# manospits/parallel_heat

Hardware: AMD Instinct MI355X
Metric: Mcells/sec (whole node) + sec/1000 iters, 8192^2 grid at 1/2/4/8 MI355X (higher is better)
Workload: dtype fp32; 1 GPU; model=heat2d 5-point Jacobi (fixed boundary), grid=8192x8192, global_batch=1, seq_len=67108864, parallelism=domain-decomp 1x1 (local), tb_depth 12, halo 12, schedule sync, converge_check=False

## Files before the change

csrc/kernels/stencil.hip:

```cpp
#include <hip/hip_runtime.h>

#include <cmath>
#include <cstdlib>
#include <cstdio>
#include <cstring>
#include <iterator>
#include <map>
#include <mutex>
#include <string>
#include <tuple>
#include <vector>

#include "heat/common.hpp"
#include "heat/init_fn.hpp"
#include "heat/kernels.hpp"
#include "tb_common.hpp"
#include "tb_exp.hpp"
#include "tb_tile.hpp"

namespace heat::gpu {
namespace {

using tbdetail::in_interior;
using tbdetail::TbArgs;
using tbdetail::TbBox;
using tbdetail::wave_max_atomic;

__global__ void init_kernel(float* base, int64_t pitch, int64_t rows, int64_t hx, int64_t hy,
                            int64_t gx0, int64_t gy0, int64_t nx, int64_t ny, int mode,
                            uint64_t seed) {
  const int64_t c = int64_t(blockIdx.x) * blockDim.x + threadIdx.x;
  if (c >= pitch) return;
  for (int64_t r = blockIdx.y; r < rows; r += gridDim.y) {
    const int64_t gx = gx0 + r - hx, gy = gy0 + c - hy;
    base[r * pitch + c] = init_value(mode, gx, gy, nx, ny, seed);
  }
}

__global__ __launch_bounds__(256) void naive_kernel(const float* __restrict__ src,
                                                    float* __restrict__ dst, StencilGeom g,
                                                    Box box, unsigned* resid) {
  const int64_t c = box.c0 + int64_t(blockIdx.x) * 64 + threadIdx.x;
  const int64_t r = box.r0 + int64_t(blockIdx.y) * 4 + threadIdx.y;
  if (tbdetail::gated(g.gate)) return;
  unsigned m = 0;
  if (r < box.r1 && c < box.c1) {
    const int64_t i = r * g.pitch + c;
    const float v = src[i];
    float out = v;
    if (in_interior(g.gx0 + r, g.nx) && in_interior(g.gy0 + c, g.ny))
      out = g.numerics == 1
                ? stencil_mpi(v, src[i - g.pitch], src[i + g.pitch], src[i - 1], src[i + 1], g.cx, g.cy)
                : stencil(v, src[i - g.pitch], src[i + g.pitch], src[i - 1], src[i + 1], g.cx, g.cy);
    dst[i] = out;
    m = __float_as_uint(fabsf(out - v));
  }
  if (resid) wave_max_atomic(m, resid);
}

__global__ void pack_kernel(const float* __restrict__ origin, int64_t pitch, Box box,
                            float* __restrict__ buf) {
  const int64_t cols = box.c1 - box.c0, n = (box.r1 - box.r0) * cols;
  for (int64_t k = int64_t(blockIdx.x) * blockDim.x + threadIdx.x; k < n;
       k += int64_t(gridDim.x) * blockDim.x) {
    const int64_t r = k / cols, c = k % cols;
    buf[k] = origin[(box.r0 + r) * pitch + box.c0 + c];
  }
}

struct BoxCopies {
  BoxCopy c[kMaxBoxCopies];
};

__global__ __launch_bounds__(128) void box_copy_kernel(float* __restrict__ origin, int64_t pitch,
                                                       BoxCopies a, int to_buf) {
  const BoxCopy& c = a.c[blockIdx.y];
  const int64_t rows = c.box.r1 - c.box.r0, cols = c.box.c1 - c.box.c0;
  for (int64_t r = blockIdx.x; r < rows; r += gridDim.x) {
    float* f = origin + (c.box.r0 + r) * pitch + c.box.c0;
    float* b = c.buf + r * cols;
    for (int64_t j = threadIdx.x; j < cols; j += blockDim.x) {
      if (to_buf) b[j] = f[j];
      else f[j] = b[j];
    }
  }
}

__global__ void unpack_kernel(const float* __restrict__ buf, float* __restrict__ origin,
                              int64_t pitch, Box box) {
  const int64_t cols = box.c1 - box.c0, n = (box.r1 - box.r0) * cols;
  for (int64_t k = int64_t(blockIdx.x) * blockDim.x + threadIdx.x; k < n;
       k += int64_t(gridDim.x) * blockDim.x) {
    const int64_t r = k / cols, c = k % cols;
    origin[(box.r0 + r) * pitch + box.c0 + c] = buf[k];
  }
}

__global__ __launch_bounds__(256) void residual_kernel(const float* __restrict__ a,
                                                       const float* __restrict__ b,
                                                       int64_t pitch, Box box, unsigned* resid) {
  const int64_t c = box.c0 + int64_t(blockIdx.x) * 64 + threadIdx.x;
  unsigned m = 0;
  if (c < box.c1)
    for (int64_t r = box.r0 + blockIdx.y * 4 + threadIdx.y; r < box.r1; r += gridDim.y * 4)
      m = max(m, __float_as_uint(fabsf(a[r * pitch + c] - b[r * pitch + c])));
  wave_max_atomic(m, resid);
}

__global__ void judge_kernel(unsigned* resids, int n, int slots, int stride, DeviceGate* gate,
                             double eps, int mpi_compat) {
  constexpr int kMax = 32;
  const int lane = threadIdx.x;
  for (int i0 = 0; i0 < n; i0 += kMax) {
    const int m = min(n - i0, kMax);
    unsigned v[kMax];
#pragma unroll
    for (int j = 0; j < kMax; ++j) v[j] = (j < m && lane < slots) ? resids[lane * stride + i0 + j] : 0u;
#pragma unroll
    for (int j = 0; j < kMax; ++j)
      if (j < m && lane < slots) resids[lane * stride + i0 + j] = 0u;
    DeviceGate gl{};
    if (lane == 0) gl = *gate;
    for (int j = 0; j < m; ++j) {
      unsigned bits = v[j];
#pragma unroll
      for (int off = 32; off >= 1; off >>= 1) bits = max(bits, unsigned(__shfl_xor(int(bits), off)));
      if (lane == 0 && gl.stop == 0u) {
        float r;
        __builtin_memcpy(&r, &bits, 4);
        const unsigned ordinal = gl.checks;
        gl.checks = ordinal + 1u;
        gl.last_bits = bits;
        unsigned why = 0u;
        if ((bits & 0x7F800000u) == 0x7F800000u) why = 2u;
        else if (mpi_compat ? double(r) <= eps : r < float(eps)) why = 1u;
        if (why) {
          gl.reason = why;
          gl.stop_check = ordinal;
          gl.stop = 1u;
        }
      }
    }
    if (lane == 0) *gate = gl;
  }
}

__device__ __forceinline__ int float_key(float f) {
  const int i = __float_as_int(f);
  return i >= 0 ? i : (i ^ 0x7FFFFFFF);
}

__global__ __launch_bounds__(256) void checksum_kernel(const float* __restrict__ origin,
                                                       int64_t pitch, int64_t lx, int64_t ly,
                                                       int64_t ox, int64_t oy, int64_t ny,
                                                       DeviceChecksum* out) {
  unsigned long long h = 0, cnt = 0;
  double sum = 0.0;
  int mn = 0x7FFFFFFF, mx = int(0x80000000);
  for (int64_t r = blockIdx.y; r < lx; r += gridDim.y) {
    const float* row = origin + r * pitch;
    const uint64_t gbase = uint64_t(ox + r) * uint64_t(ny) + uint64_t(oy);
    for (int64_t c = int64_t(blockIdx.x) * blockDim.x + threadIdx.x; c < ly;
         c += int64_t(gridDim.x) * blockDim.x) {
      const float v = row[c];
      const uint32_t bits = __float_as_uint(v);
      h += mix64((gbase + uint64_t(c)) * 0x100000001B3ull ^ bits);
      sum += double(v);
      const int k = float_key(v);
      mn = min(mn, k);
      mx = max(mx, k);
      ++cnt;
    }
  }
#pragma unroll
  for (int off = 32; off >= 1; off >>= 1) {
    h += __shfl_xor(h, off);
    cnt += __shfl_xor(cnt, off);
    sum += __shfl_xor(sum, off);
    mn = min(mn, __shfl_xor(mn, off));
    mx = max(mx, __shfl_xor(mx, off));
  }
  __shared__ unsigned long long sh_h[4], sh_c[4];
  __shared__ double sh_s[4];
  __shared__ int sh_mn[4], sh_mx[4];
  const int w = threadIdx.x >> 6;
  if ((threadIdx.x & 63) == 0) {
    sh_h[w] = h;
    sh_c[w] = cnt;
    sh_s[w] = sum;
    sh_mn[w] = mn;
    sh_mx[w] = mx;
  }
  __syncthreads();
  if (threadIdx.x == 0) {
    for (int i = 1; i < int(blockDim.x >> 6); ++i) {
      h += sh_h[i];
      cnt += sh_c[i];
      sum += sh_s[i];
      mn = min(mn, sh_mn[i]);
      mx = max(mx, sh_mx[i]);
    }
    if (cnt) {
      atomicAdd(&out->hash, h);
      atomicAdd(&out->count, cnt);
      atomicAdd(&out->sum, sum);
      atomicMin(&out->min_key, mn);
      atomicMax(&out->max_key, mx);
    }
  }
}

int grid_1d(int64_t n) { return int(std::min<int64_t>(ceil_div(n, 256), 256 * 16)); }

}

bool tb_depth_supported(int k) {
  return (k >= 1 && k <= kTbMaxDepth) || k == kTbDeepDepth;
}

int tb_strip_width(int k, int lane_cols) {
  return 64 * lane_cols - 2 * int(round_up(k, lane_cols));
}
int tb_lane_cols(int variant) { return (variant & tbv::kFloat2) ? 2 : 4; }

int tb_variant_lag(int variant) {
  const int pipe = variant & tbv::kPipeMask;
  if (pipe == tbv::kRamp && (variant & tbv::kPrefetch6)) return 4;
  switch (pipe) {
    case tbv::kRing4: return 2;
    case tbv::kRing2: return 0;
    case tbv::kRamp: return 3;
    default: return 1;
  }
}

bool tb_variant_split(int variant) {
  return (variant & tbv::kSplit) && tb_variant_deep(variant);
}

bool tb_variant_deep(int variant) {
  return (variant & tbv::kScalar) && !(variant & tbv::kFloat2) && tb_variant_lag(variant) == 3;
}

namespace {
TbTuning tuning_from_env() {
  TbTuning t;
  auto geti = [](const char* n, int def) {
    const char* e = std::getenv(n);
    return e && *e ? std::atoi(e) : def;
  };
  t.variant = geti("HEAT_TB_VARIANT", -1);
  t.rounds = std::max(0, geti("HEAT_TB_ROUNDS", 0));
  t.min_len = std::max(0, geti("HEAT_TB_MINLEN", 0));
  t.waves = std::max(0, geti("HEAT_TB_WAVES", 0));
  t.tile_rows = std::max(0, geti("HEAT_TB_TILE_ROWS", 0));
  t.tile_waves = std::max(0, geti("HEAT_TB_TILE_WAVES", 0));
  t.tile_xl = geti("HEAT_TB_TILE_XL", -1);
  t.res_diag = geti("HEAT_TB_RES_DIAG", 0) & 31;
  t.nt = geti("HEAT_TB_NT", -1);
  t.tile_max_srps = std::max(0, geti("HEAT_TB_TILE_MAX", 64));
  if (const char* e = std::getenv("HEAT_TB_EDGE_FRAC"); e && *e) t.edge_frac = std::atof(e);
  if (const char* e = std::getenv("HEAT_TB_AGE_WEIGHTS"); e && *e) {
    for (const char* q = e; *q;) {
      char* end = nullptr;
      const double v = std::strtod(q, &end);
      if (end == q) break;
      t.age_weights.push_back(v);
      q = *end == ',' ? end + 1 : end;
    }
  } else if (const char* r = std::getenv("HEAT_TB_AGE_RATIO"); r && *r) {
    t.age_weights = {std::atof(r), 1.0};
  }
  return t;
}
std::mutex g_tuning_mu;
TbTuning& tuning_ref() {
  static TbTuning t = tuning_from_env();
  return t;
}
}

TbTuning tb_tuning() {
  std::lock_guard<std::mutex> lk(g_tuning_mu);
  return tuning_ref();
}

void tb_set_tuning(const TbTuning& t) {
  std::lock_guard<std::mutex> lk(g_tuning_mu);
  tuning_ref() = t;
}

int tb_default_rounds() { return tb_tuning().rounds; }

namespace {
bool tb_trace_enabled() {
  static const bool on = [] {
    const char* e = std::getenv("HEAT_TB_TRACE");
    return e && *e && *e != '0';
  }();
  return on;
}
void tb_trace_once(const char* line) {
  static std::mutex mu;
  static std::vector<std::string> seen;
  std::lock_guard<std::mutex> lk(mu);
  for (const auto& s : seen)
    if (s == line) return;
  seen.emplace_back(line);
  std::fputs(line, stderr);
}
}

int tb_simd_count() {
  static std::map<int, int> cache;
  static std::mutex mu;
  int dev = 0;
  HIP_CHECK(hipGetDevice(&dev));
  std::lock_guard<std::mutex> lk(mu);
  auto it = cache.find(dev);
  if (it != cache.end()) return it->second;
  int cus = 0;
  HIP_CHECK(hipDeviceGetAttribute(&cus, hipDeviceAttributeMultiprocessorCount, dev));
  return cache.emplace(dev, std::max(1, cus) * 4).first->second;
}

int tb_auto_waves_per_simd(int depth, int64_t strip_rows_per_simd, int max_per_simd) {
  int w = max_per_simd;
  if (strip_rows_per_simd < 6 * int64_t(depth)) w = 1;
  else if (strip_rows_per_simd * 2 < 25 * int64_t(depth)) w = 2;
  return std::max(1, std::min(w, max_per_simd));
}

int tb_resident_waves(int depth, int variant) {
  static std::map<std::tuple<int, int, int>, int> cache;
  static std::mutex mu;
  int dev = 0;
  HIP_CHECK(hipGetDevice(&dev));
  std::lock_guard<std::mutex> lk(mu);
  auto key = std::make_tuple(dev, depth, variant);
  auto it = cache.find(key);
  if (it != cache.end()) return it->second;
  int cus = 0;
  HIP_CHECK(hipDeviceGetAttribute(&cus, hipDeviceAttributeMultiprocessorCount, dev));
  const int lag = tb_variant_lag(variant);
  if (tb_variant_split(variant)) {
    const int occ = (variant & tbv::kShiftMixed)
                        ? tb_exp("the mixed-shift split build (kShiftMixed)").tbxm_occupancy_split(depth)
                        : tbx::occupancy_split(depth);
    const int w = std::max(1, cus * std::max(1, occ) * 2);
    cache.emplace(key, w);
    return w;
  }
  const int per_cu = (variant & tbv::kFloat2)  ? tb_exp("the float2-lane build (kFloat2)").tbn_occupancy(depth, lag)
                     : (variant & tbv::kScalar) ? tbs::occupancy(depth, lag)
                                                : tb_exp("the packed build (no kScalar)").tbp_occupancy(depth, lag);
  const int w = std::max(1, cus * std::max(1, per_cu) * 4);
  cache.emplace(key, w);
  return w;
}

int tb_default_variant(int depth) {
  if (const int v = tb_tuning().variant; v >= 0) return v;
  return depth == kTbDeepDepth ? tbv::kDefaultDeep : tbv::kDefault;
}

int tb_auto_variant(int depth, int64_t strip_rows_per_simd) {
  if (const int v = tb_tuning().variant; v >= 0) return v;
  if (depth >= 4 && depth % 2 == 0 && strip_rows_per_simd < tb_tuning().tile_max_srps)
    return tbv::kTile | tbv::kXcdGroups;
  if (depth == kTbDeepDepth && strip_rows_per_simd < 64) return tbv::kDefault;
  if (depth == 8 && strip_rows_per_simd >= 256) return tbv::kDefaultDeep;
  return tb_default_variant(depth);
}

void init_field(float* origin, const Layout& L, int64_t gx0, int64_t gy0, int64_t nx, int64_t ny,
                int mode, uint64_t seed, hipStream_t st) {
  float* base = origin - L.origin();
  dim3 grid(unsigned(ceil_div(L.pitch, 256)), unsigned(std::min<int64_t>(L.rows, 1024)));
  hipLaunchKernelGGL(init_kernel, grid, dim3(256), 0, st, base, L.pitch, L.rows, int64_t(L.hx),
                     int64_t(L.hy), gx0, gy0, nx, ny, mode, seed);
  HIP_CHECK(hipGetLastError());
}

void naive_step(const float* src, float* dst, const StencilGeom& g, const Box& box,
                unsigned* resid, hipStream_t st) {
  if (box.empty()) return;
  dim3 grid(unsigned(ceil_div(box.cols(), 64)), unsigned(ceil_div(box.rows(), 4)));
  hipLaunchKernelGGL(naive_kernel, grid, dim3(64, 4), 0, st, src, dst, g, box, resid);
  HIP_CHECK(hipGetLastError());
}

namespace {
struct Stamps {
  unsigned long long* buf = nullptr;
  int64_t waves = 0;
};
std::mutex g_stamps_mu;
std::map<int, Stamps> g_stamps;

Stamps stamps_of_current_device() {
  int dev = 0;
  HIP_CHECK(hipGetDevice(&dev));
  std::lock_guard<std::mutex> lk(g_stamps_mu);
  auto it = g_stamps.find(dev);
  return it == g_stamps.end() ? Stamps{} : it->second;
}
}

void tb_set_stamps(unsigned long long* buf, int64_t waves) {
  int dev = 0;
  HIP_CHECK(hipGetDevice(&dev));
  std::lock_guard<std::mutex> lk(g_stamps_mu);
  if (buf) g_stamps[dev] = Stamps{buf, waves};
  else g_stamps.erase(dev);
}

bool tb_mid_residual(int depth) {
  return depth == kTbDeepDepth && tb_tuning().variant < 0;
}

namespace {
std::mutex g_exp_mu;
const TbExpKernels* g_exp = nullptr;
}

bool tb_exp_loaded() {
  std::lock_guard<std::mutex> lk(g_exp_mu);
  return g_exp != nullptr;
}

const TbExpKernels& tb_exp(const char* what) {
  std::lock_guard<std::mutex> lk(g_exp_mu);
  HEAT_CHECK(g_exp != nullptr,
             "%s is an experiment kernel build: `make exp`, then load "
             "parallel_heat_amd/_lib/libheat_exp.so (HEAT_EXP=1)", what);
  return *g_exp;
}

bool split_pk_enabled() {
  static const bool on = [] {
    const char* e = std::getenv("HEAT_TB_SPLIT_PK");
    return e && *e && *e != '0';
  }();
  return on;
}

constexpr int64_t kTbStreamBytes = int64_t(192) << 20;

void tb_step(const float* src, float* dst, const StencilGeom& g, const Box* boxes, int nbox,
             int depth, unsigned* resid, hipStream_t st, int waves_target, int variant,
             int res_level, TbChain* chain) {
  if (chain) chain->chained = false;
  HEAT_CHECK(nbox >= 0 && nbox <= 5, "nbox=%d", nbox);
  HEAT_CHECK(res_level >= 0 && res_level <= depth, "residual level %d of a depth-%d pass",
             res_level, depth);
  if (res_level == depth || resid == nullptr) res_level = 0;
  const bool forced = variant >= 0 || tb_tuning().variant >= 0;
  const TbTuning tune = tb_tuning();
  if (variant < 0) {
    const int W4 = tb_strip_width(depth, 4);
    int64_t rows4 = 0;
    for (int b = 0; b < nbox; ++b)
      if (!boxes[b].empty()) rows4 += ceil_div(boxes[b].cols(), W4) * boxes[b].rows();
    variant = tb_auto_variant(depth, rows4 / tb_simd_count());
    if (!tb_depth_supported(depth) && depth % 2 == 0 && depth <= 16)
      variant = tbv::kTile | tbv::kXcdGroups;
  }
  const bool tile_depth = (variant & tbv::kTile) && depth % 2 == 0 && depth <= 16;
  HEAT_CHECK(tb_depth_supported(depth) || tile_depth, "unsupported TB depth %d (variant %d)", depth,
             variant);
  if (variant & tbv::kTile) {
    if (depth % 2 == 0) {
      tbw::step(src, dst, g, boxes, nbox, depth, resid, res_level, st, variant, tune);
      return;
    }
    variant = (variant & ~(tbv::kTile | tbv::kTileDpp | 3)) | tbv::kDefault;
  }
  HEAT_CHECK(res_level == 0 || (tb_variant_split(variant) && depth == kTbDeepDepth),
             "a residual at step %d of a depth-%d pass needs the depth-12 level-split or tile "
             "kernel (variant %d%s)", res_level, depth, variant, forced ? ", forced" : "");
  const int lag = tb_variant_lag(variant);
  const int W = tb_strip_width(depth, tb_lane_cols(variant));
  int64_t total_strip_rows = 0;
  for (int b = 0; b < nbox; ++b)
    if (!boxes[b].empty()) total_strip_rows += ceil_div(boxes[b].cols(), W) * boxes[b].rows();
  const std::vector<double>& env_weights = tune.age_weights;
  const bool split_v = tb_variant_split(variant);
  int G = 0;
  std::vector<double> weights;
  auto set_weights = [&](int max_groups) {
    if (!env_weights.empty())
      weights = env_weights;
    else if (split_v)
      weights.assign(std::begin(kTbSplitAgeWeights), std::end(kTbSplitAgeWeights));
    else
      weights = {kTbAgeRatio, 1.0};
    bool uneven = false;
    for (double w : weights) uneven = uneven || w != weights[0] || w <= 0.0;
    G = uneven && int(weights.size()) >= 2 && int(weights.size()) <= max_groups ? int(weights.size()) : 0;
  };
  if (variant & tbv::kForceAgePairs) {
    set_weights(4);
    if (G == 0) {
      G = 2;
      weights.assign(2, 1.0);
    }
  }
  int bpc = 0;
  if (waves_target <= 0) {
    const int resident = tb_resident_waves(depth, variant);
    const int rounds = waves_target < 0 ? -waves_target : tune.rounds;
    if (rounds > 0) {
      waves_target = rounds * resident;
    } else {
      const int simds = tb_simd_count();
      const int per_simd = tb_auto_waves_per_simd(depth, total_strip_rows / simds,
                                                  std::max(1, resident / simds));
      waves_target = simds * per_simd;
      const int blocks_per_cu = split_v ? 2 * per_simd : per_simd;
      bpc = blocks_per_cu;
      if (G == 0 && blocks_per_cu >= 2 && !(variant & tbv::kFloat2) &&
          !(variant & tbv::kNoAgePairs))
        set_weights(blocks_per_cu);
    }
  }
  const bool pairs = G > 0;
  TbArgs args{};
  args.src = src;
  args.dst = dst;
  args.resid = resid;
  args.res_level = res_level > 0 ? res_level : depth;
  args.g = g;
  args.flags = ((variant & tbv::kXcdGroups) ? tbdetail::kTbXcdGroups : 0) |
               ((variant & tbv::kAltDirection) ? tbdetail::kTbAltDirection : 0) |
               ((variant & tbv::kDiagNoStore) ? tbdetail::kTbDiagNoStore : 0) |
               ((variant & tbv::kDiagCachedRows) ? tbdetail::kTbDiagCachedRows : 0);
  const int64_t min_len = tune.min_len > 0 ? tune.min_len : std::max<int64_t>(depth, 8);
  int64_t len = std::max<int64_t>(min_len, ceil_div(total_strip_rows, waves_target));
  const double edge_frac = tune.edge_frac;
  int n = 0, waves = 0;
  auto plan = [&](int64_t L) {
    const int64_t edge_len = std::max<int64_t>(std::min<int64_t>(min_len, L),
                                               int64_t(double(L) * edge_frac));
    n = 0;
    waves = 0;
    auto add = [&](const Box& B, int64_t clen) {
      if (B.empty()) return;
      HEAT_CHECK(n < tbdetail::kMaxBoxes, "too many TB sub-boxes");
      TbBox& t = args.box[n++];
      t.r0 = B.r0;
      t.r1 = B.r1;
      t.c0 = B.c0;
      t.c1 = B.c1;
      t.nstrips = int(ceil_div(B.cols(), W));
      t.chunk_len = int(std::min<int64_t>(clen, B.rows()));
      t.nchunks = int(ceil_div(B.rows(), t.chunk_len));
      if (pairs) {
        t.chunk_len = int(std::max<int64_t>(1, ceil_div(std::min<int64_t>(G * clen, B.rows()), G)));
        t.nchunks = int(ceil_div(B.rows(), G * int64_t(t.chunk_len)));
      }
      t.wave_begin = waves;
      waves += t.nstrips * t.nchunks * (pairs ? G : 1);
    };
    for (int b = 0; b < nbox; ++b) {
      const Box& B = boxes[b];
      if (B.empty()) continue;
      HEAT_CHECK(B.c0 % 4 == 0, "TB box column start %lld not a multiple of 4", (long long)B.c0);
      Box mid = B, top{}, bot{};
      if (edge_len < L && B.rows() > 2 * L) {
        const int64_t top_end = 1 - g.gx0 + depth;
        const int64_t bot_begin = g.nx - 2 - g.gx0 - depth;
        if (B.r0 < top_end) {
          const int64_t e = std::min(B.r1, std::max(top_end, B.r0 + edge_len));
          top = Box{B.r0, e, B.c0, B.c1};
          mid.r0 = e;
        }
        if (B.r1 - 1 > bot_begin && mid.r1 > mid.r0) {
          const int64_t s0 = std::max(mid.r0, std::min(bot_begin + 1, B.r1 - edge_len));
          bot = Box{s0, B.r1, B.c0, B.c1};
          mid.r1 = s0;
        }
      }
      add(top, edge_len);
      add(mid, L);
      add(bot, edge_len);
    }
  };
  bool linear = variant & tbv::kLinear;
  if (!linear) {
    plan(len);
    for (int it = 0; it < 8 && waves > waves_target; ++it) {
      len = std::max(len + 1, ceil_div(len * int64_t(waves), int64_t(waves_target)));
      plan(len);
    }
    linear = !(variant & tbv::kNoLinear) && waves < (9 * int64_t(waves_target)) / 10 &&
             total_strip_rows >= 32 * int64_t(depth) * waves_target;
  }
  if (linear) {
    n = 0;
    int64_t total = 0;
    for (int b = 0; b < nbox; ++b) {
      const Box& B = boxes[b];
      if (B.empty()) continue;
      HEAT_CHECK(B.c0 % 4 == 0, "TB box column start %lld not a multiple of 4", (long long)B.c0);
      TbBox& t = args.box[n++];
      t.r0 = B.r0;
      t.r1 = B.r1;
      t.c0 = B.c0;
      t.c1 = B.c1;
      t.nstrips = int(ceil_div(B.cols(), W));
      t.nchunks = 1;
      t.chunk_len = int(std::min<int64_t>(B.rows(), INT32_MAX));
      t.wave_begin = 0;
      t.lin0 = total;
      total += int64_t(t.nstrips) * B.rows();
    }
    if (n == 0) return;
    if (pairs && env_weights.empty() && split_v && bpc >= 4) {
      weights.assign(std::begin(kTbLinearAgeWeights), std::end(kTbLinearAgeWeights));
      G = int(weights.size());
    }
    const int Gl = pairs ? G : 1;
    const int64_t units = std::max<int64_t>(
        Gl, std::min<int64_t>(waves_target, total / std::max<int64_t>(1, min_len)));
    waves = int(units / Gl * Gl);
    args.lin_total = total;
    args.lin_slack = 2 * int64_t(depth);
    args.flags |= tbdetail::kTbLinear;
  }
  if (n == 0) return;
  args.nbox = n;
  args.total_waves = waves;
  if (pairs) {
    for (int b = 0; b < n; ++b) args.box[b].wave_begin /= G;
    args.total_waves = waves / G;
    args.flags |= tbdetail::kTbAgePairs;
    args.age_groups = G;
    double tot = 0.0;
    for (double w : weights) tot += w;
    double acc = 0.0;
    args.age_cum[0] = 0;
    for (int a = 0; a < G; ++a) {
      acc += weights[size_t(a)];
      args.age_cum[a + 1] = a + 1 == G ? 1024 : int(std::lround(1024.0 * acc / tot));
    }
  }
  const bool split = tb_variant_split(variant);
  if (split && !(variant & tbv::kShiftMixed)) {
    int64_t bytes = 0;
    for (int b = 0; b < nbox; ++b)
      if (!boxes[b].empty()) bytes += boxes[b].rows() * g.pitch * int64_t(sizeof(float));
    const bool nt = tune.nt >= 0 ? tune.nt != 0 : bytes > kTbStreamBytes;
    if (nt) args.flags |= tbdetail::kTbStreamRows;
  }
  if (tb_trace_enabled()) {
    char line[320];
    std::snprintf(line, sizeof line,
                  "[heat tb] depth %d variant %d boxes %d strip_rows %lld waves_target %d bpc %d "
                  "linear %d units %d age_groups %d cum %d,%d,%d,%d chunk0 %d nchunks0 %d nt %d\n",
                  depth, variant, n, (long long)total_strip_rows, waves_target, bpc,
                  int((args.flags & tbdetail::kTbLinear) != 0), waves, pairs ? G : 0,
                  args.age_cum[1], args.age_cum[2], args.age_cum[3], args.age_cum[4],
                  args.box[0].chunk_len, args.box[0].nchunks,
                  int((args.flags & tbdetail::kTbStreamRows) != 0));
    tb_trace_once(line);
  }
  if (const Stamps sb = stamps_of_current_device(); sb.buf) {
    const int64_t need = int64_t(waves) * (split ? 2 : 1);
    HEAT_CHECK(need <= sb.waves, "stamp buffer holds %lld waves, launch has %lld",
               (long long)sb.waves, (long long)need);
    args.stamps = sb.buf;
  }
  if (chain && chain->passes > 1) {
    const int G = (args.flags & tbdetail::kTbAgePairs) ? args.age_groups : 1;
    int blocks = (args.total_waves + 1) / 2;
    if (G > 1) blocks = (blocks + 7) / 8 * 8 * G;
    static const int occ = tb_exp("the chained build (HEAT_TB_CHAIN=1)").tbc_occupancy_chain(kTbDeepDepth);
    int dev = 0, cus = 0;
    HIP_CHECK(hipGetDevice(&dev));
    HIP_CHECK(hipDeviceGetAttribute(&cus, hipDeviceAttributeMultiprocessorCount, dev));
    const bool fits = split && !(variant & tbv::kShiftMixed) && (args.flags & tbdetail::kTbStreamRows) &&
                      !(args.flags & tbdetail::kTbLinear) && !(args.flags & tbdetail::kTbAltDirection) &&
                      n == 1 && resid == nullptr && depth == kTbDeepDepth && args.stamps == nullptr &&
                      int64_t(args.total_waves) * G <= chain->max_units && blocks <= cus * occ;
    if (tb_trace_enabled()) {
      char line[320];
      std::snprintf(line, sizeof line,
                    "[heat chain] passes %d split %d mixed %d stream %d linear %d alt %d boxes %d resid %d "
                    "depth %d units %d x %d max %d blocks %d cus %d occ %d -> %d\n",
                    chain->passes, int(split), int((variant & tbv::kShiftMixed) != 0),
                    int((args.flags & tbdetail::kTbStreamRows) != 0),
                    int((args.flags & tbdetail::kTbLinear) != 0),
                    int((args.flags & tbdetail::kTbAltDirection) != 0), n, int(resid != nullptr), depth,
                    args.total_waves, G, chain->max_units, blocks, cus, occ, int(fits));
      tb_trace_once(line);
    }
    if (fits) {
      chain->chained = tb_exp("the chained build (HEAT_TB_CHAIN=1)")
                           .tbc_launch_chain(args, depth, chain->passes, chain->flags, chain->done,
                                             chain->err, st);
      HIP_CHECK(hipGetLastError());
      return;
    }
  }
  bool ok;
  if (split) {
    if (variant & tbv::kShiftMixed)
      ok = tb_exp("the mixed-shift split build (kShiftMixed)").tbxm_launch_split(args, depth, st);
    else if (!(args.flags & tbdetail::kTbStreamRows))
      ok = tbx::launch_split(args, depth, st);
    else if (split_pk_enabled())
      ok = tb_exp("the packed split build (HEAT_TB_SPLIT_PK=1)").tbxnp_launch_split(args, depth, st);
    else
      ok = tbxn::launch_split(args, depth, st);
  } else if (variant & tbv::kFloat2) {
    ok = tb_exp("the float2-lane build (kFloat2)").tbn_launch(args, depth, lag, st);
  } else if (variant & tbv::kScalar) {
    ok = tbs::launch(args, depth, lag, st);
  } else {
    ok = tb_exp("the packed build (no kScalar)").tbp_launch(args, depth, lag, st);
  }
  HEAT_CHECK(ok, "TB depth %d is not instantiated for variant %d (depth %d: scalar ring-3+ramp only)",
             depth, variant, kTbDeepDepth);
  HIP_CHECK(hipGetLastError());
}

void pack_box(const float* origin, int64_t pitch, const Box& box, float* buf, hipStream_t st) {
  if (box.empty()) return;
  hipLaunchKernelGGL(pack_kernel, dim3(grid_1d(box.rows() * box.cols())), dim3(256), 0, st,
                     origin, pitch, box, buf);
  HIP_CHECK(hipGetLastError());
}

void copy_boxes(float* origin, int64_t pitch, const BoxCopy* copies, int n, bool to_buf,
                hipStream_t st) {
  HEAT_CHECK(n >= 0 && n <= kMaxBoxCopies, "copy_boxes: %d boxes", n);
  BoxCopies a{};
  int m = 0;
  int64_t rows = 0;
  for (int i = 0; i < n; ++i) {
    if (copies[i].box.empty()) continue;
    a.c[m++] = copies[i];
    rows = std::max(rows, copies[i].box.rows());
  }
  if (m == 0) return;
  dim3 grid(unsigned(std::min<int64_t>(rows, 2048)), unsigned(m));
  hipLaunchKernelGGL(box_copy_kernel, grid, dim3(128), 0, st, origin, pitch, a, int(to_buf));
  HIP_CHECK(hipGetLastError());
}

void unpack_box(const float* buf, float* origin, int64_t pitch, const Box& box, hipStream_t st) {
  if (box.empty()) return;
  hipLaunchKernelGGL(unpack_kernel, dim3(grid_1d(box.rows() * box.cols())), dim3(256), 0, st,
                     buf, origin, pitch, box);
  HIP_CHECK(hipGetLastError());
}

float checksum_key_to_float(int key) {
  const int i = key >= 0 ? key : (key ^ 0x7FFFFFFF);
  float f;
  std::memcpy(&f, &i, 4);
  return f;
}

void checksum_block(const float* origin, int64_t pitch, int64_t lx, int64_t ly, int64_t ox,
                    int64_t oy, int64_t ny, DeviceChecksum* out, hipStream_t st) {
  if (lx <= 0 || ly <= 0) return;
  const int64_t gx = std::min<int64_t>(ceil_div(ly, 256), 16);
  dim3 grid(unsigned(gx), unsigned(std::min<int64_t>(lx, std::max<int64_t>(1, 2048 / gx))));
  hipLaunchKernelGGL(checksum_kernel, grid, dim3(256), 0, st, origin, pitch, lx, ly, ox, oy, ny,
                     out);
  HIP_CHECK(hipGetLastError());
}

void judge_check(unsigned* resid, DeviceGate* gate, double eps, bool mpi_compat, hipStream_t st,
                 int n, int slots, int stride) {
  HEAT_CHECK(n >= 1 && slots >= 1 && slots <= 64 && (slots == 1 || stride >= n),
             "judge of %d checks x %d slots", n, slots);
  hipLaunchKernelGGL(judge_kernel, dim3(1), dim3(64), 0, st, resid, n, slots, stride, gate, eps,
                     int(mpi_compat));
  HIP_CHECK(hipGetLastError());
}

void residual_box(const float* a, const float* b, int64_t pitch, const Box& box, unsigned* resid,
                  hipStream_t st) {
  if (box.empty()) return;
  dim3 grid(unsigned(ceil_div(box.cols(), 64)),
            unsigned(std::min<int64_t>(ceil_div(box.rows(), 4), 1024)));
  hipLaunchKernelGGL(residual_kernel, grid, dim3(64, 4), 0, st, a, b, pitch, box, resid);
  HIP_CHECK(hipGetLastError());
}

}

extern "C" void heat_register_exp_kernels(const heat::gpu::TbExpKernels* k) {
  std::lock_guard<std::mutex> lk(heat::gpu::g_exp_mu);
  heat::gpu::g_exp = k;
}
```

csrc/kernels/tb_resident.hip:

```cpp
#include <algorithm>
#include <cstdio>
#include <cstdlib>
#include <map>
#include <mutex>
#include <set>
#include <string>
#include <tuple>

#include "heat/common.hpp"
#include "heat/plan.hpp"
#include "tb_resident_kern.hpp"

namespace heat::gpu::tbw {

bool res_launch_x0(const ResArgs& ra, int rows, int waves, int blocks, hipStream_t st);
bool res_launch_x1(const ResArgs& ra, int rows, int waves, int blocks, hipStream_t st);
bool res_launch_x2(const ResArgs& ra, int rows, int waves, int blocks, hipStream_t st);
int res_occupancy_x0(int rows, int waves);
int res_occupancy_x1(int rows, int waves);
int res_occupancy_x2(int rows, int waves);

namespace {
int occupancy_res(int rows, int waves, int xl) {
  return xl == 1 ? res_occupancy_x1(rows, waves)
         : xl == 2 ? res_occupancy_x2(rows, waves)
                   : res_occupancy_x0(rows, waves);
}

bool launch_res(const ResArgs& ra, int rows, int waves, int xl, int blocks, hipStream_t st) {
  return xl == 1 ? res_launch_x1(ra, rows, waves, blocks, st)
         : xl == 2 ? res_launch_x2(ra, rows, waves, blocks, st)
                   : res_launch_x0(ra, rows, waves, blocks, st);
}

int cached_occupancy_res(int rows, int waves, int xl) {
  static std::map<std::tuple<int, int, int, int>, int> cache;
  static std::mutex mu;
  int dev = 0;
  HIP_CHECK(hipGetDevice(&dev));
  std::lock_guard<std::mutex> lk(mu);
  const auto key = std::make_tuple(dev, rows, waves, xl);
  auto it = cache.find(key);
  if (it != cache.end()) return it->second;
  return cache.emplace(key, occupancy_res(rows, waves, xl)).first->second;
}

struct ResPlan {
  int rows = 0, waves = 0, units = 0;
};

int res_xl(int variant, const TbTuning& tune) {
  if (tune.tile_xl >= 0 && tune.tile_xl <= 2) return tune.tile_xl;
  return variant >= 0 && (variant & tbv::kTileDpp) ? 0 : 2;
}

ResPlan plan_res(const Box& box, int depth, int xl, const TbTuning& tune) {
  ResPlan best;
  if (box.empty() || depth < 4 || depth % 2 != 0 || box.c0 % 4 != 0) return best;
  const int W = tb_strip_width(depth, 4);
  const int cus = tb_simd_count() / 4;
  double best_est = 0.0;
  struct Shape {
    int rows, waves;
  };
  static constexpr Shape kShapes[] = {{12, 8}, {13, 8}, {14, 8}, {16, 8}, {20, 8}, {24, 8}, {12, 16}, {20, 16}};
  for (const Shape& sh : kShapes) {
    if (tune.tile_rows > 0 && sh.rows != tune.tile_rows) continue;
    if (tune.tile_waves > 0 && sh.waves != tune.tile_waves) continue;
    const int64_t hmax = int64_t(sh.waves) * sh.rows - 2 * int64_t(depth);
    if (hmax < std::max(depth, 4)) continue;
    const int64_t units = ceil_div(box.cols(), W) * ceil_div(box.rows(), hmax);
    const int occ = cached_occupancy_res(sh.rows, sh.waves, xl);
    if (occ <= 0 || units > int64_t(cus) * occ) continue;
    const double est = tile_step_estimate(units, cus, occ, sh.rows, sh.waves);
    if (best.rows == 0 || est < best_est) {
      best_est = est;
      best = ResPlan{sh.rows, sh.waves, int(units)};
    }
  }
  return best;
}
}

}

namespace heat::gpu {

bool tb_resident_fits(const Box& box, int depth, int variant) {
  using namespace tbw;
  const TbTuning tune = tb_tuning();
  const ResPlan pl = plan_res(box, depth, res_xl(variant, tune), tune);
  if (pl.rows == 0) return false;
  const int64_t hmax = int64_t(pl.waves) * pl.rows - 2 * int64_t(depth);
  const int64_t n = ceil_div(box.rows(), hmax);
  return ceil_div(box.rows(), n) >= depth;
}

int tb_resident_shape(const Box& box, int depth, int variant) {
  using namespace tbw;
  const TbTuning tune = tb_tuning();
  const ResPlan pl = plan_res(box, depth, res_xl(variant, tune), tune);
  if (pl.rows == 0) return 0;
  const int64_t hmax = int64_t(pl.waves) * pl.rows - 2 * int64_t(depth);
  if (ceil_div(box.rows(), ceil_div(box.rows(), hmax)) < depth) return 0;
  return res_shape(pl.rows, pl.waves);
}

void tb_resident_step(const float* src, float* dst, const StencilGeom& g, const Box& box,
                      int depth, int passes, const TbResidentBuffers& xb, hipStream_t st,
                      int variant, const TbResidentCheck* checks, int nchecks, unsigned* resids,
                      int64_t own_rows, int64_t own_cols) {
  using namespace tbw;
  HEAT_CHECK(passes >= 2, "a resident launch spans >= 2 passes (%d)", passes);
  const TbTuning tune = tb_tuning();
  int xl = res_xl(variant, tune);
  const ResPlan pl = plan_res(box, depth, xl, tune);
  HEAT_CHECK(pl.rows > 0, "resident tiles do not fit box %lldx%lld at depth %d",
             (long long)box.rows(), (long long)box.cols(), depth);
  HEAT_CHECK(pl.units <= xb.max_tiles, "%d resident tiles, flag buffer holds %d", pl.units,
             xb.max_tiles);
  HEAT_CHECK(xb.bytes < (int64_t(1) << 31), "exchange field of %lld bytes (32-bit offsets)",
             (long long)xb.bytes);
  const int64_t hmax = int64_t(pl.waves) * pl.rows - 2 * int64_t(depth);
  ResArgs ra{};
  TbArgs& a = ra.a;
  a.src = src;
  a.dst = dst;
  HEAT_CHECK(nchecks >= 0 && nchecks <= kResMaxChecks && (nchecks == 0 || resids != nullptr),
             "%d checks in a resident launch (at most %d)", nchecks, kResMaxChecks);
  for (int c = 0; c < nchecks; ++c) {
    HEAT_CHECK(checks[c].pass >= 0 && checks[c].pass < passes && checks[c].step >= 2 &&
                   checks[c].step <= depth && checks[c].step % 2 == 0 &&
                   (c == 0 || checks[c].pass > checks[c - 1].pass),
               "resident check %d at pass %d step %d (passes %d, depth %d)", c, checks[c].pass,
               checks[c].step, passes, depth);
    ra.chk_pass[c] = checks[c].pass;
    ra.chk_step[c] = checks[c].step;
  }
  ra.nchk = nchecks;
  ra.resids = resids;
  a.resid = nchecks > 0 ? resids : nullptr;
  static const bool diag_res1 = [] {
    const char* e = std::getenv("HEAT_TB_RES_DIAG_RES1");
    return e && *e && *e != '0';
  }();
  if (diag_res1 && resids) a.resid = resids;
  if (variant < 0 && tune.tile_xl < 0 && pl.rows <= kTilePkRows &&
      cached_occupancy_res(pl.rows, pl.waves, 0) >= cached_occupancy_res(pl.rows, pl.waves, xl))
    xl = 0;
  a.res_level = depth;
  a.g = g;
  a.flags = (variant < 0 || (variant & tbv::kXcdGroups)) ? tbdetail::kTbXcdGroups : 0;
  TbBox& t = a.box[0];
  t.r0 = box.r0;
  t.r1 = box.r1;
  t.c0 = box.c0;
  t.c1 = box.c1;
  t.nstrips = int(ceil_div(box.cols(), tb_strip_width(depth, 4)));
  t.nchunks = int(ceil_div(box.rows(), hmax));
  t.chunk_len = int(ceil_div(box.rows(), int64_t(t.nchunks)));
  HEAT_CHECK(t.chunk_len >= depth, "resident tiles of %d rows at depth %d", t.chunk_len, depth);
  t.wave_begin = 0;
  a.nbox = 1;
  a.total_waves = t.nstrips * t.nchunks;
  HEAT_CHECK(a.total_waves == pl.units, "resident plan %d != %d tiles", pl.units, a.total_waves);
  ra.passes = passes;
  ra.depth = depth;
  ra.xbase[0] = xb.base[0];
  ra.xbase[1] = xb.base[1];
  ra.xorigin = xb.origin;
  ra.xbytes = int(xb.bytes);
  HEAT_CHECK(xb.done != nullptr, "resident launch without a completion counter");
  ra.flags = xb.flags;
  ra.done = xb.done;
  ra.err = xb.err;
  ra.own_r1 = nchecks > 0 ? own_rows : box.r1;
  ra.own_c1 = nchecks > 0 ? own_cols : box.c1;
  ra.diag = tune.res_diag;
  if (const char* e = std::getenv("HEAT_TB_TRACE"); e && *e && *e != '0') {
    static std::mutex mu;
    static std::set<std::string> seen;
    char line[200];
    std::snprintf(line, sizeof line, "[heat tb] resident depth %d passes %d rows %d waves %d xl %d tiles %d\n",
                  depth, passes, pl.rows, pl.waves, xl, pl.units);
    std::lock_guard<std::mutex> lk(mu);
    if (seen.insert(line).second) std::fputs(line, stderr);
  }
  HEAT_CHECK(launch_res(ra, pl.rows, pl.waves, xl, pl.units, st), "resident %dx%d not built",
             pl.rows, pl.waves);
  HIP_CHECK(hipGetLastError());
}

}
```

csrc/kernels/tb_resident_kern.hpp:

```cpp
#pragma once

#include <algorithm>
#include <type_traits>

#include "heat/common.hpp"
#include "tb_tile.hpp"
#include "tb_tile_core.hpp"

namespace heat::gpu::tbw {

constexpr int kResMaxChecks = kTbResidentMaxChecks;

struct ResArgs {
  TbArgs a;
  int passes;
  int depth;
  float* xbase[2];
  int64_t xorigin;
  int xbytes;
  unsigned* flags;
  unsigned* done;
  unsigned* err;
  int64_t own_r1, own_c1;
  int nchk;
  unsigned* resids;
  int chk_pass[kResMaxChecks], chk_step[kResMaxChecks];
  int diag;
};

constexpr unsigned kSpinLimit = 1u << 22;

__device__ __forceinline__ void wave_max_atomic_u(float m, unsigned* word) {
  unsigned mm = __float_as_uint(m);
#pragma unroll
  for (int off = 32; off >= 1; off >>= 1) mm = max(mm, unsigned(__shfl_xor(int(mm), off)));
  if ((threadIdx.x & 63) == 0) atomicMax(word, mm);
}

template <int R, int NW, int MODE, int XL, int RES>
__device__ __forceinline__ void resident_run(const ResArgs& ra, const TbBox& bx, int strip, int t,
                                             int u, vecf (*xch)[2][NW][64]) {
  const TbArgs& a = ra.a;
  const int K = ra.depth;
  const int lane = threadIdx.x & 63;
  const int w = __builtin_amdgcn_readfirstlane(threadIdx.x >> 6);
  const StencilGeom& g = a.g;
  const int KK = (K + 3) & ~3;
  const int64_t Wd = 256 - 2 * KK;
  const int64_t cbase = bx.c0 + int64_t(strip) * Wd;
  const int64_t cend = min(cbase + Wd, bx.c1);
  const int64_t col = cbase - KK + 4 * lane;
  const bool store_lane = col >= cbase && col < cend;
  const int rc = int(min<int64_t>(cend - col, 4));
  const int64_t ub = bx.r0 + int64_t(t) * bx.chunk_len;
  const int64_t ue = min(ub + bx.chunk_len, bx.r1);
  const int64_t row0 = ub - K + int64_t(w) * R;
  const int64_t rmin = bx.r0 - K, rmax = bx.r1 + K - 1;
  const int64_t pitch = g.pitch;
  const float* __restrict__ src = a.src + (cbase - KK);
  float* __restrict__ dst = a.dst + (cbase - KK);
  const int lo = 4 * lane;

  Tile<R, MODE, RES, XL> T;
  auto ld = [&](int r) {
    int64_t row = min(max(row0 + r, rmin), rmax);
    opaque(row);
    return *reinterpret_cast<const vecf*>(src + row * pitch + lo);
  };
  T.u[0] = ld(0);
  T.u[R - 1] = ld(R - 1);
#pragma unroll
  for (int r = 1; r < R - 1; ++r) T.u[r] = ld(r);

  Upd<MODE, XL> up;
  up.cx = to_vgpr(g.cx);
  up.cy = to_vgpr(g.cy);
  auto bits = [](int64_t lo_r, int64_t hi_r) -> unsigned {
    const int l = int(max<int64_t>(0, min<int64_t>(lo_r, R)));
    const int h = int(max<int64_t>(0, min<int64_t>(hi_r, R)));
    const unsigned top = h >= 32 ? ~0u : (1u << h) - 1u;
    return l >= h ? 0u : top & ~((1u << l) - 1u);
  };
  unsigned rowmask;
  tile_mode_setup(up, g, col, bits(1 - (g.gx0 + row0), g.nx - 1 - (g.gx0 + row0)), rowmask);
  unsigned usemask = bits(ub - row0, ue - row0);
  const unsigned bandmask = usemask & (bits(ub - row0, ub + K - row0) | bits(ue - K - row0, ue - row0));
  const unsigned ghostmask =
      bits(max(ub - K, bx.r0) - row0, ub - row0) | bits(ue - row0, min(ue + K, bx.r1) - row0);
  const bool band_lane = store_lane && (col < cbase + KK || col + 4 > cend - KK);
  const bool ghost_lane = !store_lane && col >= bx.c0 && col < bx.c1;
  const bool box_lane = col >= bx.c0 && col < bx.c1;
  const unsigned resmask = bits(max<int64_t>(ub, 0) - row0, min<int64_t>(ue, ra.own_r1) - row0);
  const int res_rc = store_lane && col >= 0 && col < ra.own_c1 ? int(min<int64_t>(ra.own_c1 - col, 4)) : 0;
  __amdgpu_buffer_rsrc_t xr[2];
#pragma unroll
  for (int i = 0; i < 2; ++i) xr[i] = __builtin_amdgcn_make_buffer_rsrc(ra.xbase[i], 0, ra.xbytes, 0x00020000);
  const int vlane = 16 * lane;
  const int xrow0 = int((ra.xorigin + row0 * pitch + (cbase - KK)) * 4);
  const int xpitch = int(pitch * 4);

  const int wa = w > 0 ? w - 1 : 0, wb = w < NW - 1 ? w + 1 : NW - 1;
  TileXc<NW> xc{xch, w, lane, 1, 0, 0, vecf{}};

  struct Pub {
    __amdgpu_buffer_rsrc_t rs;
    unsigned usemask, bandmask;
    int vs, vb;
    int xrow0, xpitch;
    __device__ __forceinline__ void row(int r, const vecf& v, const vecf&) {
      const int vo = ((usemask >> r) & 1u) ? (((bandmask >> r) & 1u) ? vs : vb) : kNoStore;
      __builtin_amdgcn_raw_buffer_store_b128(__builtin_bit_cast(u32x4, v), rs, vo, xrow0 + r * xpitch,
                                             16);
    }
  };

  float pend_m = 0.f;
  int pend_c = -1;
  int next_chk = 0;
  auto flush_resid = [&]() {
    if constexpr (RES == 1) {
      if (pend_c >= 0) {
        const int slot = (u * NW + w) & (kTbResidentSlots - 1);
        wave_max_atomic_u(pend_m, ra.resids + slot * kResMaxChecks + pend_c);
        pend_c = -1;
      }
    }
  };

  auto pass = [&](auto last_c, int p) {
    constexpr bool LAST = decltype(last_c)::value;
    xch[1][0][w][lane] = T.u[R - 1];
    xch[1][1][w][lane] = T.u[0];
    lds_barrier();
    xc.efirst = xch[1][0][wa][lane];
    int xr0 = xrow0, xp = xpitch;
    opaque32(xr0);
    opaque32(xp);
    const bool nopub = ra.diag & 4;
    unsigned pum = nopub ? 0u : usemask, pbm = bandmask;
    opaque(pum);
    opaque(pbm);
    Pub pub{xr[p & 1], pum, pbm, store_lane ? vlane : kNoStore, band_lane ? vlane : kNoStore, xr0, xp};
    int64_t off0 = row0 * pitch;
    opaque(off0);
    RowStoreSink fin{dst + off0, pitch, pum, store_lane ? vlane : kNoStore};
    int ci = -1;
    if constexpr (RES == 1) {
      if (next_chk < ra.nchk && ra.chk_pass[next_chk] == p) ci = next_chk++;
    }
    int acc_step = ci >= 0 ? ra.chk_step[ci] - 1 : -1;
    opaque32(acc_step);
    unsigned rm = ci >= 0 ? resmask : 0u;
    opaque(rm);
    tile_pass_steps<RES == 1 ? 3 : 0, 3>(
        K,
        [&](auto down_c, auto what_c, auto acc_c, int s) {
          constexpr bool D = decltype(down_c)::value;
          xc.p = s & 1;
          xc.last_w = xc.next_w = D ? wb : wa;
          const vecf first_nb = xc.efirst;
          opaque(rowmask);
          opaque(usemask);
          const unsigned rms = s == acc_step ? rm : 0u;
          if constexpr (LAST)
            T.template step<D, decltype(what_c)::value, decltype(acc_c)::value>(
                first_nb, xc, up, rowmask, usemask, store_lane, rc, &fin,
                rms, res_rc);
          else
            T.template step<D, decltype(what_c)::value, decltype(acc_c)::value>(
                first_nb, xc, up, rowmask, usemask, store_lane, rc, &pub,
                rms, res_rc);
        },
        acc_step);
    if constexpr (RES == 1) {
      if constexpr (R > 16) asm volatile("" : "+v"(T.m));
      if (ci >= 0) {
        pend_m = T.m;
        pend_c = ci;
        T.m = 0.f;
        if constexpr (LAST) flush_resid();
      }
    }
  };

  auto refill = [&](int p) {
    if (w == 0 && !(ra.diag & 1)) {
      const int ns = bx.nstrips, nc = bx.nchunks;
      const int ds = lane < 3 ? -1 : lane < 5 ? 0 : 1;
      const int dt = (lane == 0 || lane == 3 || lane == 5) ? -1 : (lane == 1 || lane == 6) ? 0 : 1;
      const int s2 = strip + ds, t2 = t + dt;
      const bool real = lane < 8 && s2 >= 0 && s2 < ns && t2 >= 0 && t2 < nc;
      const unsigned* f = ra.flags + (real ? s2 * nc + t2 : u);
      for (unsigned spins = 0;; ++spins) {
        const unsigned v =
            real ? __hip_atomic_load(f, __ATOMIC_RELAXED, __HIP_MEMORY_SCOPE_AGENT) : unsigned(p);
        if (__all(v >= unsigned(p))) break;
        if (spins >= kSpinLimit) {
          if (lane == 0) __hip_atomic_fetch_or(ra.err, 1u, __ATOMIC_RELAXED, __HIP_MEMORY_SCOPE_AGENT);
          break;
        }
        __builtin_amdgcn_s_sleep(2);
      }
    }
    __syncthreads();
    if (ra.diag & 2) {
      flush_resid();
      return;
    }
    const __amdgpu_buffer_rsrc_t rs = xr[(p - 1) & 1];
    unsigned gm = ghostmask, um = usemask;
    opaque(gm);
    opaque(um);
    int xr0 = xrow0, xp = xpitch;
    opaque32(xr0);
    opaque32(xp);
#pragma unroll
    for (int r = 0; r < R; ++r) {
      const bool full = (gm >> r) & 1u;
      const bool part = (um >> r) & 1u;
      if ((full && box_lane) || (part && ghost_lane))
        T.u[r] = __builtin_bit_cast(vecf, __builtin_amdgcn_raw_buffer_load_b128(rs, vlane, xr0 + r * xp, 16));
    }
    flush_resid();
  };

  const int P = ra.passes;
  for (int p = 0; p + 1 < P; ++p) {
    if (p > 0) refill(p);
    pass(std::false_type{}, p);
    asm volatile("s_waitcnt vmcnt(0)" ::: "memory");
    __syncthreads();
    if (threadIdx.x == 0)
      __hip_atomic_store(ra.flags + u, unsigned(p + 1), __ATOMIC_RELAXED, __HIP_MEMORY_SCOPE_AGENT);
  }
  refill(P - 1);
  pass(std::true_type{}, P - 1);
}

template <int R, int NW, int XL, int RES>
__global__ __launch_bounds__(64 * NW, (tile_waves_per_simd<R, NW>())) void tile_resident_kernel(
    ResArgs ra) {
  __shared__ vecf xch[2][2][NW][64];
  const TbArgs& a = ra.a;
  if (tbdetail::gated(a.g.gate)) return;
  int blk = blockIdx.x;
  if (a.flags & tbdetail::kTbXcdGroups) {
    const int nb = gridDim.x, q = nb >> 3, r = nb & 7, x = blk & 7, j = blk >> 3;
    blk = x * q + min(x, r) + j;
  }
  const TbBox& bx = a.box[0];
  const int strip = blk / bx.nchunks, t = blk % bx.nchunks;
  const StencilGeom& g = a.g;
  const int K = ra.depth, KK = (K + 3) & ~3;
  const int64_t cbase = bx.c0 + int64_t(strip) * (256 - 2 * KK);
  const int64_t gy_lo = g.gy0 + cbase - KK, gy_hi = gy_lo + 255;
  const int64_t ub = bx.r0 + int64_t(t) * bx.chunk_len;
  const int64_t wx_lo = g.gx0 + ub - K + int64_t(__builtin_amdgcn_readfirstlane(threadIdx.x >> 6)) * R;
  const int64_t wx_hi = wx_lo + R - 1;
  const int mode = (ra.diag & 8) ? kTileGeneric : tile_mode(g, wx_lo, wx_hi, gy_lo, gy_hi, ra.diag & 16);
  tile_dispatch<XL, (RES == 0 && R <= kTilePkRows)>(mode, [&](auto mode_c) {
    resident_run<R, NW, decltype(mode_c)::value, XL, RES>(ra, bx, strip, t, blk, xch);
    return 0.f;
  });
  __shared__ unsigned last;
  __syncthreads();
  if (threadIdx.x == 0) {
    const unsigned n = __hip_atomic_fetch_add(ra.done, 1u, __ATOMIC_ACQ_REL, __HIP_MEMORY_SCOPE_AGENT);
    last = n + 1 == unsigned(gridDim.x);
  }
  __syncthreads();
  if (last) {
    for (int i = threadIdx.x; i < int(gridDim.x); i += blockDim.x)
      __hip_atomic_store(ra.flags + i, 0u, __ATOMIC_RELAXED, __HIP_MEMORY_SCOPE_AGENT);
    if (threadIdx.x == 0) __hip_atomic_store(ra.done, 0u, __ATOMIC_RELAXED, __HIP_MEMORY_SCOPE_AGENT);
  }
}

template <class Kern>
int occ_kernel(Kern k, int NW) {
  int n = 0;
  if (hipOccupancyMaxActiveBlocksPerMultiprocessor(&n, k, 64 * NW, 0) != hipSuccess) n = 1;
  hipFuncAttributes fa{};
  if (hipFuncGetAttributes(&fa, reinterpret_cast<const void*>(k)) == hipSuccess && fa.numRegs > 0) {
    const int alloc = (fa.numRegs + 7) / 8 * 8;
    n = std::min(n, (512 / alloc) / (NW / 4));
  }
  return std::max(0, n);
}

template <int R, int NW, int XL>
int occ_res() {
  return std::min(occ_kernel(tile_resident_kernel<R, NW, XL, 0>, NW),
                  occ_kernel(tile_resident_kernel<R, NW, XL, 1>, NW));
}

#define HEAT_RES_SHAPES(X) X(12, 8) X(13, 8) X(14, 8) X(16, 8) X(20, 8) X(24, 8) X(12, 16) X(20, 16)

template <int R, int NW, int XL>
void launch_res_x(const ResArgs& ra, int blocks, hipStream_t st) {
  if (ra.a.resid != nullptr)
    hipLaunchKernelGGL((tile_resident_kernel<R, NW, XL, 1>), dim3(blocks), dim3(64 * NW), 0, st, ra);
  else
    hipLaunchKernelGGL((tile_resident_kernel<R, NW, XL, 0>), dim3(blocks), dim3(64 * NW), 0, st, ra);
}

template <int XL>
bool res_launch_unit(const ResArgs& ra, int rows, int waves, int blocks, hipStream_t st) {
#define HEAT_RES_CASE(r, nw)                     \
  if (rows == r && waves == nw) {                \
    launch_res_x<r, nw, XL>(ra, blocks, st);     \
    return true;                                 \
  }
  HEAT_RES_SHAPES(HEAT_RES_CASE)
#undef HEAT_RES_CASE
  return false;
}

template <int XL>
int res_occupancy_unit(int rows, int waves) {
#define HEAT_RES_CASE(r, nw) \
  if (rows == r && waves == nw) return occ_res<r, nw, XL>();
  HEAT_RES_SHAPES(HEAT_RES_CASE)
#undef HEAT_RES_CASE
  return 0;
}

}
```

Before: 5.116 million Mcells/s.

## Gather resident-tile column ghosts with packed lane loads and LDS redistribution

The refill step now loads box rows as before, but fetches the partial-row column ghosts differently. Instead of one b128 load per ghost row issued only from the few ghost lanes, lanes are remapped so that each of NL loads covers ghost columns across many rows at once. The gathered values are then scattered through the LDS exchange buffer back to the owning ghost lanes. This cuts the number of mostly-empty vector memory instructions per refill, at the cost of an extra LDS round trip, a ballot/popcount mapping and a new depth limit (ghost lanes <= 6). One shape (R=16, XL=2) keeps the old path, and a diag bit selects a probe variant.

```diff
diff --git a/csrc/kernels/stencil.hip b/csrc/kernels/stencil.hip
--- a/csrc/kernels/stencil.hip
+++ b/csrc/kernels/stencil.hip
@@ -256,7 +256,7 @@
   t.tile_rows = std::max(0, geti("HEAT_TB_TILE_ROWS", 0));
   t.tile_waves = std::max(0, geti("HEAT_TB_TILE_WAVES", 0));
   t.tile_xl = geti("HEAT_TB_TILE_XL", -1);
-  t.res_diag = geti("HEAT_TB_RES_DIAG", 0) & 31;
+  t.res_diag = geti("HEAT_TB_RES_DIAG", 0) & 63;
   t.nt = geti("HEAT_TB_NT", -1);
   t.tile_max_srps = std::max(0, geti("HEAT_TB_TILE_MAX", 64));
   if (const char* e = std::getenv("HEAT_TB_EDGE_FRAC"); e && *e) t.edge_frac = std::atof(e);
diff --git a/csrc/kernels/tb_resident.hip b/csrc/kernels/tb_resident.hip
--- a/csrc/kernels/tb_resident.hip
+++ b/csrc/kernels/tb_resident.hip
@@ -122,6 +122,9 @@
   HEAT_CHECK(xb.bytes < (int64_t(1) << 31), "exchange field of %lld bytes (32-bit offsets)",
              (long long)xb.bytes);
   const int64_t hmax = int64_t(pl.waves) * pl.rows - 2 * int64_t(depth);
+  HEAT_CHECK(((depth + 3) & ~3) / 2 <= kResGhostLanes,
+             "resident tiles gather the column ghosts of depth <= %d (%d)", 2 * kResGhostLanes,
+             depth);
   ResArgs ra{};
   TbArgs& a = ra.a;
   a.src = src;
diff --git a/csrc/kernels/tb_resident_kern.hpp b/csrc/kernels/tb_resident_kern.hpp
--- a/csrc/kernels/tb_resident_kern.hpp
+++ b/csrc/kernels/tb_resident_kern.hpp
@@ -27,6 +27,14 @@
   int chk_pass[kResMaxChecks], chk_step[kResMaxChecks];
   int diag;
 };
+
+constexpr int kResGhostLanes = 6;
+
+__device__ __forceinline__ int int_to_vgpr(int x) {
+  int r;
+  asm("v_mov_b32 %0, %1" : "=v"(r) : "s"(x));
+  return r;
+}
 
 constexpr unsigned kSpinLimit = 1u << 22;
 
@@ -214,12 +222,62 @@
     int xr0 = xrow0, xp = xpitch;
     opaque32(xr0);
     opaque32(xp);
-#pragma unroll
-    for (int r = 0; r < R; ++r) {
-      const bool full = (gm >> r) & 1u;
-      const bool part = (um >> r) & 1u;
-      if ((full && box_lane) || (part && ghost_lane))
-        T.u[r] = __builtin_bit_cast(vecf, __builtin_amdgcn_raw_buffer_load_b128(rs, vlane, xr0 + r * xp, 16));
+    if (gm != 0) {
+#pragma unroll
+      for (int r = 0; r < R; ++r)
+        if (((gm >> r) & 1u) && box_lane)
+          T.u[r] = __builtin_bit_cast(vecf, __builtin_amdgcn_raw_buffer_load_b128(rs, vlane, xr0 + r * xp, 16));
+    }
+    if constexpr (R == 16 && XL == 2 && RES == 1) {
+#pragma unroll
+      for (int r = 0; r < R; ++r)
+        if (((um >> r) & 1u) && ghost_lane)
+          T.u[r] = __builtin_bit_cast(vecf, __builtin_amdgcn_raw_buffer_load_b128(rs, vlane, xr0 + r * xp, 16));
+      flush_resid();
+      return;
+    }
+    constexpr int GPS = 64 / R, NL = (kResGhostLanes + GPS - 1) / GPS;
+    int ln = 0;
+    asm volatile("" : "+v"(ln));
+    ln = __builtin_amdgcn_mbcnt_hi(~0u, __builtin_amdgcn_mbcnt_lo(~0u, ln));
+    const unsigned long long gb = __ballot(ghost_lane);
+    unsigned gbw = unsigned(gb), gbe = unsigned(gb >> 32);
+    asm volatile("" : "+s"(gbw), "+s"(gbe));
+    const int nW = int_to_vgpr(__builtin_popcount(gbw));
+    const int G = min(nW + int_to_vgpr(__builtin_popcount(gbe)), NL * GPS);
+    const int eL = int_to_vgpr(gbe ? 32 + __builtin_ctz(gbe) : 64);
+    const int rlo = um ? __builtin_ctz(um) : 0;
+    const int gj = ln / R, rj = ln - gj * R;
+    const bool rowok = gj < GPS && ((um >> rj) & 1u);
+    const int rowoff = (rj - rlo) * xp;
+    xr0 += rlo * xp;
+    vecf gv[NL];
+    if (ra.diag & 32) {
+#pragma unroll
+      for (int i = 0; i < NL; ++i) {
+        gv[i] = __builtin_bit_cast(vecf, __builtin_amdgcn_raw_buffer_load_b128(
+                                             rs, box_lane ? 16 * ln : kNoStore, xr0 + i * xp, 16));
+        asm volatile("" ::"v"(gv[i]));
+      }
+    } else {
+#pragma unroll
+      for (int i = 0; i < NL; ++i) {
+        const int gq = i * GPS + gj;
+        const int pl = gq < nW ? gq : eL + gq - nW;
+        gv[i] = __builtin_bit_cast(vecf, __builtin_amdgcn_raw_buffer_load_b128(
+                                             rs, rowok && gq < G ? 16 * pl + rowoff : kNoStore, xr0, 16));
+      }
+#pragma unroll
+      for (int i = 0; i < NL; ++i) xch[i >> 1][i & 1][w][lane] = gv[i];
+      asm volatile("s_waitcnt lgkmcnt(0)" ::: "memory");
+      const int gi = ln < 32 ? ln : nW + ln - eL;
+      if (ghost_lane && gi < G) {
+        const int slot = gi / GPS;
+        const vecf* const mine = &xch[0][0][w][lane] + (slot * (NW * 64) + (gi - slot * GPS) * R - ln);
+#pragma unroll
+        for (int r = 0; r < R; ++r)
+          if ((um >> r) & 1u) T.u[r] = mine[r];
+      }
     }
     flush_resid();
   };
```

Result: no change. 5.115 million Mcells/s (-0.0%).
